# michaelfeil/skyjo_rl

Measured on AMD Instinct MI355X. Metric: env-steps/sec (whole node) at 65 536 parallel 3-player games, higher is better.
Workload: dtype int8

## Files before the change

skyjo_rl_amd/csrc/skyjo_step.h:

```cpp
#pragma once
#ifndef SKYJO_DEVICE_PARTS
#error "include skyjo_device.h"
#endif

__device__ __forceinline__ void sk_publish_deals(const SkParams &P, int g) {
  const size_t G = (size_t)P.tiles * SK_TILE;
  const int b = P.busy[g];
  if (b) {
    const uint32_t tag = P.plan_tag[g];
    const uint32_t f = __hip_atomic_load(&P.done_flag[g], __ATOMIC_RELAXED, __HIP_MEMORY_SCOPE_AGENT);
    if ((f & 0x7fffffffu) == tag) {
      SK_FENCE_ACQUIRE(P);
      if (!P.cancel[g] && f == tag) P.spare_ready[(size_t)(b - 1) * G + g] = 1;
      P.busy[g] = 0, P.cancel[g] = 0;
    }
  }
}
__device__ __forceinline__ void sk_plan_deals(const SkParams &P, int g, int lane) {
  const size_t G = (size_t)P.tiles * SK_TILE;
  bool need = false, empty = false;
  if (g < P.B) {
    const uint8_t busy = P.busy[g];
    const int head = P.bank_head[g] % SK_BANK;
    const uint32_t consumed = P.deals_consumed[g];
    uint8_t ready[SK_BANK];
#pragma unroll
    for (int k = 0; k < SK_BANK; k++) ready[k] = P.spare_ready[(size_t)k * G + g];
    bool open = true;
    int r = 0;
#pragma unroll
    for (int k = 0; k < SK_BANK; k++) {
      uint8_t f = 0;
#pragma unroll
      for (int j = 0; j < SK_BANK; j++) f = (head + k) % SK_BANK == j ? ready[j] : f;
      open = open && f != 0;
      r += open ? 1 : 0;
    }
    need = !busy && r < SK_BANK;
    empty = need && r == 0;
    if (need) {
      P.busy[g] = (uint8_t)(1 + (head + r) % SK_BANK);
      P.cancel[g] = 0;
      P.plan_ep[g] = consumed + (uint32_t)r;
      P.plan_tag[g] = P.plan_new_tag;
    }
  }
  const unsigned long long be = __ballot(empty);
  if (be && lane == 0) atomicAdd(P.bank_empty + (P.be_add & 1u), (uint32_t)__popcll(be));
}

__device__ __forceinline__ void sk_error_to_host(const SkParams &P, int lane) {
  if (lane == 0) {
    const uint32_t e = __hip_atomic_load(P.dev_error, __ATOMIC_RELAXED, __HIP_MEMORY_SCOPE_AGENT);
    if (e) P.health_host[2] = e;
  }
}
__device__ __forceinline__ void sk_export_raw(const SkParams &P, uint8_t *lp, int g, uint8_t *o) {
  for (int c = 0; c < P.L.chunks; c++) ((uint4 *)o)[c] = LQ(c);
  double *d = (double *)(o + P.L.state_bytes);
  for (int p = 0; p < P.L.N; p++) d[p] = P.rewards[(size_t)g * P.L.N + p], d[P.L.N + p] = P.scores[(size_t)g * P.L.N + p];
  uint32_t *m = (uint32_t *)(d + 2 * P.L.N);
  m[0] = P.rng_mode == SKYJO_RNG_MT19937 ? (uint32_t)P.mt_idx[g] : 0u;
  m[1] = P.done[g];
}

__device__ __forceinline__ uint32_t sk_next_tag(uint32_t t) {
  t = (t + 1u) & 0x7fffffffu;
  return t ? t : 1u;
}
template <bool INDIRECT, bool POLICY, int NP, bool PLANAR = false>
__device__ __forceinline__ void step_body(const SkParams &Pin, const int tile, const int lane, uint32_t *lds_raw, const int32_t *actions,
                                          uint8_t *rec_out, int32_t *act_out, int iters, uint64_t policy_seed, uint64_t iter0,
                                          double *end_rew_out, uint8_t *end_out, uint8_t *raw_out, int raw_stride, const int cycle_len = 0,
                                          const bool defer_ok = true) {
  SkParams P = Pin;
  TRACE_DECL;
  if (NP > 0) P.L = sk_make_layout(NP, INDIRECT ? 1 : 0);
  const int g = tile * SK_TILE + lane;
  const uint32_t lds_tile = (uint32_t)(uintptr_t)(__attribute__((address_space(3))) uint32_t *)lds_raw;
  uint8_t *lp = (uint8_t *)lds_raw + lane * 16;
  uint8_t *stg = (uint8_t *)lds_raw + P.L.chunks * 1024;
  uint8_t *fp = stg + lane * 4;
  const int stg_bytes = (INDIRECT || PLANAR) ? 4096 : SK_TILE * (P.L.rec_bytes + 16);
  uint8_t *ap = stg + stg_bytes + lane * 8;
  constexpr bool DEFER = POLICY && NP > 0 && NP < 8;
  constexpr bool REGACC = NP > 0 && NP < 8;
  constexpr int NACC = REGACC ? SK_ACC_KINDS * NP : 1;
  double racc_store[NACC];
#pragma unroll
  for (int k = 0; k < NACC; k++) racc_store[k] = 0.0;
  double *racc = REGACC ? racc_store : nullptr;
  uint8_t *pendp = DEFER && defer_ok ? stg + stg_bytes + (REGACC ? 0 : SK_ACC_KINDS * P.L.N * 512) + lane * 16 : nullptr;
  int pend_fin = -1;
  if (!REGACC)
    for (int k = 0; k < SK_ACC_KINDS * P.L.N; k++) ACC(k) = 0.0;
  STAMP_DECL;
  if (!POLICY) tile_load(P, P.state, tile, lane, lp);
  else dma_record<true>((const uint8_t *)P.state, (uint32_t)((((size_t)tile * P.L.chunks) * SK_TILE + lane) * 16), lds_tile, P.L.chunks);
  if (P.ov_flags & 1u) sk_publish_deals(P, g);
  sk_vm_drain();
  HdrRegs h;
  HDR_LOAD(h);
  STAMP(0);
  const bool valid = ((h.w0 >> 16) & F_VALID) != 0;
  LaneCounters cnt;
  uint32_t r0 = 0, r1 = 0, r2 = 0, r3 = 0;
  const uint64_t gid = P.game_id0 + (uint64_t)g;
  ObsRegs ob;
  if (valid) obs_load(P, lp, (h.w0 >> 8) & 0xff, ob);
  for (int it = 0; it < iters; it++) {
    const uint64_t iter = iter0 + (uint64_t)it;
    if (POLICY && (it == 0 || (iter & 3) == 0)) {
      philox4x32_10((uint32_t)(iter >> 2), (uint32_t)gid, (uint32_t)(gid >> 32), 0x504F4C00u, (uint32_t)policy_seed,
                    (uint32_t)(policy_seed >> 32), r0, r1, r2, r3);
      for (int k = (int)(iter & 3); k > 0; k--) {
        const uint32_t t = r0;
        r0 = r1, r1 = r2, r2 = r3, r3 = t;
      }
    }
    STAMP_T(3);
    const uint32_t word = r0;
    if (POLICY) {
      r0 = r1, r1 = r2, r2 = r3, r3 = word;
    }
    int a = -1;
    if (valid) {
      const bool over = ((h.w0 >> 16) & F_DONE) != 0;
      if (!POLICY) a = actions[g];
      const bool skip = !POLICY && a == SKYJO_ACTION_SKIP;
      const bool acted = !over && !skip;
      SpareRegs sp;
      const bool resetting = over && P.auto_reset && !skip;
      if (resetting) spare_issue(P, lp, lds_tile, tile, lane, g, sp);
      STAMP_T(4);
      if (!over && !skip) {
        const uint32_t v0 = ob.q0, v1 = ob.q1, v2 = ob.q2;
        STAMP_N(2);
        const uint4 row_pre = LQ(sk_pb(P.L, (h.w0 >> 8) & 0xff) >> 4);
        asm volatile("" ::: "memory");
        if (POLICY) a = policy_pick(h.w0 & 0xff, ob, word);
#ifndef SK_STAMPS_FINE
        STAMP_N(3);
#endif
        apply_action<INDIRECT, NP, POLICY>(P, lp, fp, ap, h, v0, v1, v2, a, g, cnt, st, pendp, pend_fin, row_pre, racc);
#ifdef SK_STAMPS_FINE
        STAMP(6);
#else
        STAMP(5);
#endif
      } else if (!skip) {
        a = -1;
        if (P.auto_reset) {
          bool dealt = true;
          if (!spare_commit(P, lp, g, sp)) {
            dealt = deal_inline(P, lp, fp, g, tile, lane, sp.head);
            cnt.waits++;
          }
          HDR_LOAD(h);
          if (SK_OFTEN(dealt)) {
            h.w0 = (h.w0 & 0x00ffffffu) | ((uint32_t)SKYJO_ST_RESET << 24);
            cnt.resets++;
          }
        } else {
          h.w0 = (h.w0 & 0x00ffffffu) | ((uint32_t)SKYJO_ST_NOOP_DONE << 24);
        }
        STAMP(1);
      } else {
        a = -1;
      }
      if (!POLICY && acted && (unsigned)a >= (unsigned)SKYJO_NUM_ACTIONS) a = -2;
      if (!POLICY && end_out) {
        const bool end = acted && ((h.w0 >> 16) & F_DONE) != 0;
        end_out[g] = end ? 1 : 0;
        for (int q = 0; q < P.L.N; q++) end_rew_out[(size_t)g * P.L.N + q] = end ? P.rewards[(size_t)g * P.L.N + q] : 0.0;
      }
      const uint4 rec_a = LQ(1);
      const uint32_t rec_b = LB(32);
      const uint4 rec_row = LQ((sk_pb(P.L, (h.w0 >> 8) & 0xff) + PB_VIS) >> 4);
      asm volatile("" ::: "memory");
      obs_from_row(rec_row, ob);
      if (rec_out) {
        if (INDIRECT) {
          uint4 rr[4];
          emit_record<INDIRECT>(P, lp, h, ob, a, nullptr, rr, &rec_a, rec_b);
          if (PLANAR) {
            typedef uint32_t u32x4_t __attribute__((ext_vector_type(4)));
            uint8_t *blk = rec_out + ((size_t)it * P.tiles + (size_t)tile) * (SK_TILE * 64) + lane * 16;
#pragma unroll
            for (int p = 0; p < 4; p++) __builtin_nontemporal_store((u32x4_t){rr[p].x, rr[p].y, rr[p].z, rr[p].w}, (u32x4_t *)(blk + p * 1024));
          } else {
#pragma unroll
            for (int p = 0; p < 4; p++) *(uint4 *)(stg + lane * 64 + ((p + (lane >> 1)) & 3) * 16) = rr[p];
          }
        } else if (PLANAR) {
          constexpr int PIECES = NP > 0 ? (((19 + 12 * NP + 3) & ~3) + 32 + 15) / 16 : 1;
          uint32_t wbuf[4 * PIECES];
#pragma unroll
          for (int k = 0; k < 4 * PIECES; k++) wbuf[k] = 0u;
          emit_record<INDIRECT>(P, lp, h, ob, a, (uint8_t *)wbuf, nullptr, &rec_a, rec_b);
          typedef uint32_t u32x4_t __attribute__((ext_vector_type(4)));
          uint8_t *blk = rec_out + ((size_t)it * P.tiles + (size_t)tile) * (SK_TILE * 16 * PIECES) + lane * 16;
#pragma unroll
          for (int p = 0; p < PIECES; p++)
            __builtin_nontemporal_store((u32x4_t){wbuf[4 * p], wbuf[4 * p + 1], wbuf[4 * p + 2], wbuf[4 * p + 3]}, (u32x4_t *)(blk + p * 1024));
        } else {
          emit_record<INDIRECT>(P, lp, h, ob, a, stg + lane * sk_stage_stride(P.L.rec_bytes), nullptr, &rec_a, rec_b);
        }
      }
      if (act_out) __builtin_nontemporal_store(a, &act_out[(size_t)it * P.B + g]);
#ifdef SK_STAMPS_FINE
      STAMP(7);
#else
      STAMP(6);
#endif
    }
    if (DEFER && ((it & (SK_SCORE_EVERY - 1)) == SK_SCORE_EVERY - 1 || it == iters - 1)) {
      if (SK_RARE(__any(pend_fin >= 0))) {
        if (pend_fin >= 0) {
          finish_game_fixed<(NP > 0 && NP < 8) ? NP : 1>(P, pendp, 1024, ap, g, pend_fin, racc);
          pend_fin = -1;
        }
      }
    }
    if (!INDIRECT && !PLANAR && rec_out) {
      typedef uint32_t u32x4_t __attribute__((ext_vector_type(4)));
      const int pieces = P.L.rec_bytes >> 4, stride = sk_stage_stride(P.L.rec_bytes);
      uint8_t *blk = rec_out + ((size_t)it * P.B + (size_t)tile * SK_TILE) * (size_t)P.L.rec_bytes;
      const int live = P.B - tile * SK_TILE;
      for (int q0 = lane; q0 < pieces * SK_TILE; q0 += 4 * SK_TILE) {
        uint4 v[4];
#pragma unroll
        for (int j = 0; j < 4; j++) {
          const int q = q0 + j * SK_TILE, r = q / pieces, p = q - r * pieces;
          if (q < pieces * SK_TILE) v[j] = *(const uint4 *)(stg + r * stride + p * 16);
        }
        if (SK_OFTEN(live >= SK_TILE)) {
#pragma unroll
          for (int j = 0; j < 4; j++) {
            const int q = q0 + j * SK_TILE;
            if (q0 - lane + j * SK_TILE < pieces * SK_TILE)
              __builtin_nontemporal_store((u32x4_t){v[j].x, v[j].y, v[j].z, v[j].w}, (u32x4_t *)(blk + (size_t)q * 16));
          }
        } else {
#pragma unroll
          for (int j = 0; j < 4; j++) {
            const int q = q0 + j * SK_TILE, r = q / pieces;
            if (q < pieces * SK_TILE && r < live)
              __builtin_nontemporal_store((u32x4_t){v[j].x, v[j].y, v[j].z, v[j].w}, (u32x4_t *)(blk + (size_t)q * 16));
          }
        }
      }
    }
    if (INDIRECT && !PLANAR && rec_out) {
      typedef uint32_t u32x4_t __attribute__((ext_vector_type(4)));
      uint8_t *blk = rec_out + ((size_t)it * P.B + (size_t)tile * SK_TILE) * 64;
      const int live = P.B - tile * SK_TILE;
      uint4 v[4];
#pragma unroll
      for (int j = 0; j < 4; j++) {
        const int r = 16 * j + (lane >> 2), p = lane & 3;
        v[j] = *(const uint4 *)(stg + r * 64 + ((p + (r >> 1)) & 3) * 16);
      }
      if (SK_OFTEN(live >= SK_TILE)) {
#pragma unroll
        for (int j = 0; j < 4; j++)
          __builtin_nontemporal_store((u32x4_t){v[j].x, v[j].y, v[j].z, v[j].w}, (u32x4_t *)(blk + j * 1024 + lane * 16));
      } else {
#pragma unroll
        for (int j = 0; j < 4; j++)
          if (16 * j + (lane >> 2) < live)
            __builtin_nontemporal_store((u32x4_t){v[j].x, v[j].y, v[j].z, v[j].w}, (u32x4_t *)(blk + j * 1024 + lane * 16));
      }
    }
    STAMP_T(2);
    if (POLICY && cycle_len && it + 1 < iters && (it + 1) % cycle_len == 0) {
      if (P.busy[g]) (void)wait_deal_done(P, g);
      sk_publish_deals(P, g);
      sk_plan_deals(P, g, lane);
      P.plan_new_tag = sk_next_tag(P.plan_new_tag);
      TRACE_WAIT_BEGIN;
      __syncthreads();
      TRACE_WAIT_END;
    }
  }
  HDR_FLUSH(h);
  tile_store_nt(P, P.state, tile, lane, lp);
  if (!POLICY && raw_out && valid) sk_export_raw(P, lp, g, raw_out + (size_t)g * raw_stride);
  if (P.ov_flags & 2u) {
    if (P.ov_flags & 1u) {
      if (P.busy[g]) (void)wait_deal_done(P, g);
      sk_publish_deals(P, g);
    }
    sk_plan_deals(P, g, lane);
  }
  if (!POLICY) {
    sk_error_to_host(P, lane);
    if (P.host_seq) {
      __threadfence_system();
      if (lane == 0) __hip_atomic_store(&P.health_host[3], P.host_seq, __ATOMIC_RELEASE, __HIP_MEMORY_SCOPE_SYSTEM);
    }
  }
  uint32_t v[7] = {cnt.steps, cnt.episodes, cnt.illegal, cnt.resets, cnt.sum_len, cnt.reshuffles, cnt.waits};
#pragma unroll
  for (int k = 0; k < 7; k++)
    for (int off = 32; off > 0; off >>= 1) v[k] += __shfl_down(v[k], off, 64);
  if (lane == 0) {
    unsigned long long *c = P.tile_counters + (size_t)tile * 8;
#pragma unroll
    for (int k = 0; k < 7; k++) c[k] += v[k];
  }
  if (__any(cnt.episodes | cnt.illegal)) {
    double mine = 0.0;
    if (REGACC) {
#pragma unroll
      for (int k = 0; k < NACC; k++) {
        double x = racc_store[k];
        for (int off = 32; off > 0; off >>= 1) x += __shfl_down(x, off, 64);
        x = __shfl(x, 0, 64);
        mine = lane == k ? x : mine;
      }
    } else {
      for (int k = 0; k < SK_ACC_KINDS * P.L.N; k++) {
        double x = ACC(k);
        for (int off = 32; off > 0; off >>= 1) x += __shfl_down(x, off, 64);
        x = __shfl(x, 0, 64);
        mine = lane == k ? x : mine;
      }
    }
    if (lane < SK_ACC_KINDS * P.L.N)
      P.acc_tile[(size_t)tile * SK_ACC_KINDS * SKYJO_MAX_PLAYERS + (lane / P.L.N) * SKYJO_MAX_PLAYERS + lane % P.L.N] += mine;
  }
  STAMP(7);
  STAMP_STORE;
  TRACE_STORE(0, (uint32_t)(iter0 / (uint64_t)(iters > 0 ? iters : 1)), lane, tile);
}

template <bool INDIRECT, bool POLICY, int NP, bool PLANAR = false>
__global__ __launch_bounds__(SK_TILE) void k_step(SkParams Pin, const int32_t *actions, uint8_t *rec_out,
                                                  int32_t *act_out, int iters, uint64_t policy_seed, uint64_t iter0,
                                                  double *end_rew_out, uint8_t *end_out, uint8_t *raw_out, int raw_stride) {
  extern __shared__ uint32_t lds_raw[];
  step_body<INDIRECT, POLICY, NP, PLANAR>(Pin, (int)blockIdx.x, (int)threadIdx.x, lds_raw, actions, rec_out, act_out, iters, policy_seed, iter0,
                                          end_rew_out, end_out, raw_out, raw_stride);
}

template <bool INDIRECT>
__device__ __forceinline__ void sk_emit_to(const SkParams &P, uint8_t *lp, const HdrRegs &h, const ObsRegs &ob, uint8_t *rec_out, int tile, int lane,
                                           int planar) {
  const int g = tile * SK_TILE + lane;
  if (INDIRECT && planar) {
    uint4 rr[4];
    emit_record<INDIRECT>(P, lp, h, ob, -1, nullptr, rr);
    uint4 *o = (uint4 *)(rec_out + (size_t)tile * SK_TILE * P.L.rec_bytes) + lane;
#pragma unroll
    for (int k = 0; k < 4; k++) o[k * SK_TILE] = rr[k];
  } else {
    emit_record<INDIRECT>(P, lp, h, ob, -1, rec_out + (size_t)g * P.L.rec_bytes);
  }
}

template <bool INDIRECT>
__global__ __launch_bounds__(SK_TILE) void k_observe(SkParams P, const int32_t *players, uint8_t *rec_out, int planar) {
  extern __shared__ uint32_t lds_raw[];
  const int tile = blockIdx.x, lane = threadIdx.x, g = tile * SK_TILE + lane;
  uint8_t *lp = (uint8_t *)lds_raw + lane * 16;
  sk_error_to_host(P, lane);
  tile_load(P, P.state, tile, lane, lp);
  if (!(LB(H_FLAGS) & F_VALID)) return;
  HdrRegs h;
  HDR_LOAD(h);
  int q = players ? players[g] : LB(H_PLAYER);
  q = q < 0 ? 0 : (q >= P.L.N ? P.L.N - 1 : q);
  ObsRegs ob;
  obs_load(P, lp, q, ob);
  sk_emit_to<INDIRECT>(P, lp, h, ob, rec_out, tile, lane, planar);
}

template <bool INDIRECT>
__global__ __launch_bounds__(SK_TILE) void k_reset(SkParams P, const uint8_t *mask, uint8_t *rec_out, uint8_t *raw_out, int raw_stride, int planar) {
  extern __shared__ uint32_t lds_raw[];
  const int tile = blockIdx.x, lane = threadIdx.x, g = tile * SK_TILE + lane;
  uint8_t *lp = (uint8_t *)lds_raw + lane * 16;
  uint8_t *fp = (uint8_t *)lds_raw + P.L.chunks * 1024 + lane * 4;
  if (g >= P.B) return;
  const bool want = !mask || mask[g];
  bool want_counted = false;
  tile_load(P, P.state, tile, lane, lp);
  if (want) {
    const int head = P.bank_head[g] % SK_BANK;
    bool dealt = true;
    if (!consume_spare(P, lp, tile, lane, g, head)) dealt = deal_inline(P, lp, fp, g, tile, lane, head);
    if (dealt) LB(H_STATUS) = SKYJO_ST_RESET;
    want_counted = dealt;
  }
  HdrRegs h;
  HDR_LOAD(h);
  if (rec_out) {
    ObsRegs ob;
    obs_load(P, lp, LB(H_PLAYER), ob);
    sk_emit_to<INDIRECT>(P, lp, h, ob, rec_out, tile, lane, planar);
  }
  if (want) tile_store(P, P.state, tile, lane, lp);
  if (raw_out && (LB(H_FLAGS) & F_VALID)) sk_export_raw(P, lp, g, raw_out + (size_t)g * raw_stride);
  sk_error_to_host(P, lane);
  const unsigned long long wb = __ballot(want_counted);
  if (want_counted && lane == __ffsll((long long)wb) - 1) P.tile_counters[(size_t)tile * 8 + 3] += __popcll(wb);
}
```

skyjo_rl_amd/csrc/skyjo_transition.h:

```cpp
#pragma once
#ifndef SKYJO_DEVICE_PARTS
#error "include skyjo_device.h"
#endif

__device__ __forceinline__ void refresh_minima(const SkParams &P, uint8_t *lp) {
  int ms = LSH(sk_pb(P.L, 0) + PB_SUM), mh = LB(sk_pb(P.L, 0) + PB_HIDDEN);
  for (int q = 1; q < P.L.N; q++) {
    int s = LSH(sk_pb(P.L, q) + PB_SUM), h = LB(sk_pb(P.L, q) + PB_HIDDEN);
    ms = s < ms ? s : ms, mh = h < mh ? h : mh;
  }
  LB(H_MINSUM) = (uint8_t)(int8_t)(ms < 127 ? ms : 127);
  LB(H_MINHID) = (uint8_t)mh;
}

template <class Rng>
__device__ __forceinline__ void reshuffle_discard(const SkParams &P, uint8_t *lp, Rng &r) {
  const int n = LB(H_NDISC), role = LB(H_ROLE), pb = P.L.off_pile;
  const int reg = role ? 0 : 1;
  for (int i = n - 1; i >= 1; i--) {
    int j = (int)rng_interval(r, (uint32_t)i);
    int ai = pb + pile_addr(reg, i), aj = pb + pile_addr(reg, j);
    uint8_t t = LB(ai);
    LB(ai) = LB(aj), LB(aj) = t;
  }
  for (int k = 0; k < n - 1; k++) LB(H_HIST + 2 + LI(pb + pile_addr(reg, k)))--;
  int last = LI(pb + pile_addr(reg, n - 1));
  LB(pb + pile_addr(reg ^ 1, 0)) = (uint8_t)last;
  LB(H_NDRAW) = (uint8_t)(n - 1), LB(H_NDISC) = 1, LB(H_ROLE) = (uint8_t)(role ^ 1);
  LB(H_TOP) = (uint8_t)last;
  int rs = LB(H_RESH);
  LB(H_RESH) = (uint8_t)(rs < 255 ? rs + 1 : 255);
}

#define SK_WAIT_OK 0
#define SK_WAIT_GAVE_UP 1
#define SK_WAIT_TIMEOUT 2
__device__ __forceinline__ int wait_deal_done(const SkParams &P, int g) {
  uint32_t f = 0;
  const uint32_t tag = P.plan_tag[g];
  for (int spin = 0; spin < (1 << P.spin_log2); spin++) {
    f = __hip_atomic_load(&P.done_flag[g], __ATOMIC_RELAXED, __HIP_MEMORY_SCOPE_AGENT);
    if ((f & 0x7fffffffu) == tag) break;
    __builtin_amdgcn_s_sleep(32);
  }
  if ((f & 0x7fffffffu) != tag) {
    atomicOr(P.dev_error, SK_ERR_DEAL_TIMEOUT);
    return SK_WAIT_TIMEOUT;
  }
  SK_FENCE_ACQUIRE(P);
  return (f >> 31) != 0 ? SK_WAIT_GAVE_UP : SK_WAIT_OK;
}

__device__ __forceinline__ uint32_t mt_untwist_y(const uint32_t *mt, int i) {
  uint32_t t = mt[i] ^ mt[i + 397 >= 624 ? i + 397 - 624 : i + 397];
  const uint32_t odd = t >> 31;
  t ^= odd ? 0x9908b0dfu : 0u;
  return (t << 1) | odd;
}
__device__ __forceinline__ void mt_untwist(uint32_t *mt, int from, int to) {
  for (int i = to; i != from;) {
    const int nx = i == 624 ? 0 : i;
    i = nx == 0 ? 623 : nx - 1;
    const uint32_t y = mt_untwist_y(mt, i);
    const int ip1 = i == 623 ? 0 : i + 1;
    mt[ip1] = (mt[ip1] & 0x80000000u) | (y & 0x7fffffffu);
    mt[i] = y & 0x80000000u;
  }
}

__device__ __forceinline__ int mt_rollback(const SkParams &P, uint32_t *mt, int g, int slot, int packed) {
  const size_t G = (size_t)P.tiles * SK_TILE;
  const int snap = P.mt_idx[(size_t)(1 + slot) * G + g];
  int from = (snap & 0xffff) + (snap >> 16), to = (packed & 0xffff) + (packed >> 16);
  from = from >= 624 ? from - 624 : from, to = to >= 624 ? to - 624 : to;
  mt_untwist(mt, from, to);
  return snap;
}

__device__ __forceinline__ void reshuffle_dispatch(const SkParams &P, uint8_t *lp, uint8_t *fp, int g) {
  if (P.rng_mode == SKYJO_RNG_MT19937) {
    const size_t G = (size_t)P.tiles * SK_TILE;
    uint32_t *mt = P.mt + (size_t)g * 624;
    const int head = LB(H_BANK) % SK_BANK;
    const int busy = P.busy[g];
    const bool inflight = busy && !P.cancel[g];
    bool undo_inflight = false;
    if (inflight) {
      const int w = wait_deal_done(P, g);
      if (w == SK_WAIT_TIMEOUT) {
        LB(H_FLAGS) |= F_DONE, LB(H_STATUS) = SKYJO_ST_ERROR, LB(H_NDRAW) = 1;
        P.done[g] = 1;
        for (int q = 0; q < P.L.N; q++) P.rewards[(size_t)g * P.L.N + q] = 0.0;
        return;
      }
      undo_inflight = w == SK_WAIT_OK;
      P.cancel[g] = 1;
    }
    int packed = P.mt_idx[g];
    if (undo_inflight) packed = mt_rollback(P, mt, g, busy - 1, packed);
    for (int k = SK_BANK - 1; k >= 0; k--) {
      const int slot = (head + k) % SK_BANK;
      if (P.spare_ready[(size_t)slot * G + g]) {
        packed = mt_rollback(P, mt, g, slot, packed);
        P.spare_ready[(size_t)slot * G + g] = 0;
      }
    }
    MtStream<16> r;
    r.open(mt, packed, fp);
    reshuffle_discard(P, lp, r);
    P.mt_idx[g] = r.close();
  } else {
    PhiloxStream r;
    r.open(P.seeds[g] + 1, *(uint32_t *)(lp + LIDX(H_EPISODE)), LB(H_RESH), 1u);
    reshuffle_discard(P, lp, r);
  }
}

#define ACC(k) (*(double *)(ap + ((k) << 9)))
__device__ __forceinline__ void acc_add(uint8_t *ap, int k, double v) {
  __hip_atomic_fetch_add(&ACC(k), v, __ATOMIC_RELAXED, __HIP_MEMORY_SCOPE_WAVEFRONT);
}
__device__ __forceinline__ void acc_episode(uint8_t *ap, int N, int p, double score, double reward, int refunded) {
  acc_add(ap, p, score), acc_add(ap, N + p, reward), acc_add(ap, 2 * N + p, reward * reward);
  if (refunded) acc_add(ap, 3 * N + p, (double)refunded);
}

__device__ __forceinline__ void finish_game(const SkParams &P, uint8_t *lp, uint8_t *fp, uint8_t *ap, int g,
                                            int finisher) {
  const int N = P.L.N;
  double *sc = P.scores + (size_t)g * N, *rw = P.rewards + (size_t)g * N;
  int mn = 0, fs = 0;
  for (int p = 0; p < N; p++) {
    int s = 0;
    for (int c = 0; c < 4; c++) {
      int b = sk_pb(P.L, p) + PB_CARDS + 3 * c;
      int t0 = LI(b), t1 = LI(b + 1), t2 = LI(b + 2);
      if (!(t0 == t1 && t1 == t2)) s += t0 + t1 + t2;
    }
    MT_FIFO(p) = (uint32_t)s;
    mn = (p == 0 || s < mn) ? s : mn;
    fs = p == finisher ? s : fs;
  }
  const bool penal = mn != fs;
#define SCORE(p) ((penal && (p) == finisher) ? (double)(int)MT_FIFO(p) * P.score_penalty : (double)(int)MT_FIFO(p))
  double sum;
  if (N < 8) {
    sum = 0.0;
    for (int p = 0; p < N; p++) sum += SCORE(p);
  } else {
    sum = ((SCORE(0) + SCORE(1)) + (SCORE(2) + SCORE(3))) + ((SCORE(4) + SCORE(5)) + (SCORE(6) + SCORE(7)));
    for (int p = 8; p < N; p++) sum += SCORE(p);
  }
  const double mean = sum / (double)N;
  for (int p = 0; p < N; p++) {
    const double d = SCORE(p);
    double r = (-d + mean) + P.mean_reward;
    const int rf = LB(sk_pb(P.L, p) + PB_REFUNDED);
    if (P.reward_refunded != 0.0) r += (double)rf * P.reward_refunded;
    sc[p] = d, rw[p] = r;
    acc_episode(ap, N, p, d, r, rf);
  }
#undef SCORE
  P.done[g] = 1;
}

template <int NP>
__device__ __forceinline__ void finish_game_fixed(const SkParams &P, const uint8_t *rows, int stride, uint8_t *ap, int g, int finisher,
                                                  double *racc = nullptr) {
  double *sc = P.scores + (size_t)g * NP, *rw = P.rewards + (size_t)g * NP;
  int s[NP], refunded[NP];
  int mn = 0, fs = 0;
#pragma unroll
  for (int p = 0; p < NP; p++) {
    const uint4 row = *(const uint4 *)(rows + p * stride);
    const uint32_t c0 = row.x, c1 = row.y, c2 = row.z;
    refunded[p] = (int)(row.w >> 24);
    const uint32_t tri[4] = {c0 & 0xffffffu, (c0 >> 24) | ((c1 & 0xffffu) << 8), (c1 >> 16) | ((c2 & 0xffu) << 16), c2 >> 8};
    int t = 0;
#pragma unroll
    for (int c = 0; c < 4; c++) {
      const int t0 = (int)(int8_t)tri[c], t1 = (int)(int8_t)(tri[c] >> 8), t2 = (int)(int8_t)(tri[c] >> 16);
      t += (t0 == t1 && t1 == t2) ? 0 : t0 + t1 + t2;
    }
    s[p] = t;
    mn = (p == 0 || t < mn) ? t : mn;
    fs = p == finisher ? t : fs;
  }
  const bool penal = mn != fs;
  double d[NP], sum = 0.0;
#pragma unroll
  for (int p = 0; p < NP; p++) {
    d[p] = (penal && p == finisher) ? (double)s[p] * P.score_penalty : (double)s[p];
    sum += d[p];
  }
  const double mean = sum / (double)NP;
#pragma unroll
  for (int p = 0; p < NP; p++) {
    double r = (-d[p] + mean) + P.mean_reward;
    if (P.reward_refunded != 0.0) r += (double)refunded[p] * P.reward_refunded;
    sc[p] = d[p], rw[p] = r;
    if (racc) {
      racc[p] += d[p], racc[NP + p] += r, racc[2 * NP + p] += r * r, racc[3 * NP + p] += (double)refunded[p];
    } else {
      acc_episode(ap, NP, p, d[p], r, refunded[p]);
    }
  }
}

struct HdrRegs {
  uint32_t w0, w1, w2;
};
#define HDR_LOAD(h) ((h).w0 = LW(0), (h).w1 = LW(1), (h).w2 = LW(2))
#define HDR_FLUSH(h) (LW(0) = (h).w0, LW(1) = (h).w1, LW(2) = (h).w2)

__device__ __forceinline__ int byte3(uint32_t a, uint32_t b, uint32_t c, int k) {
  const uint32_t w = k < 4 ? a : (k < 8 ? b : c);
  return (int)(int8_t)(w >> ((k & 3) * 8));
}
__device__ __forceinline__ void put3(uint32_t &a, uint32_t &b, uint32_t &c, int k, int val) {
  const uint32_t sh = (uint32_t)(k & 3) * 8u, m = ~(0xffu << sh), v = ((uint32_t)val & 0xffu) << sh;
  if (k < 4) a = (a & m) | v;
  else if (k < 8) b = (b & m) | v;
  else c = (c & m) | v;
}
__device__ __forceinline__ void hist_add(uint8_t *lp, int value, int delta) {
  const int b = H_HIST + 2 + value;
  uint32_t *w = (uint32_t *)(lp + LIDX(b & ~3));
  const uint32_t d = (uint32_t)delta << ((b & 3) * 8);
  __hip_atomic_fetch_add(w, d, __ATOMIC_RELAXED, __HIP_MEMORY_SCOPE_WAVEFRONT);
}
__device__ __forceinline__ uint32_t swar_nonzero01(uint32_t x) {
  return ((((x & 0x7f7f7f7fu) + 0x7f7f7f7fu) | x) & 0x80808080u) >> 7;
}
__device__ __forceinline__ uint32_t pack12(uint32_t a, uint32_t b, uint32_t c) {
  return ((a * 0x00204081u >> 21) & 0xfu) | (((b * 0x00204081u >> 21) & 0xfu) << 4) |
         (((c * 0x00204081u >> 21) & 0xfu) << 8);
}

struct ObsRegs {
  uint32_t q0, q1, q2, nz0, nz1, nz2, hd0, hd1, hd2;
};
__device__ __forceinline__ void obs_from_row(const uint4 &row, ObsRegs &o) {
  o.q0 = row.x, o.q1 = row.y, o.q2 = row.z;
  o.nz0 = swar_nonzero01(o.q0 ^ 0xf2f2f2f2u);
  o.nz1 = swar_nonzero01(o.q1 ^ 0xf2f2f2f2u);
  o.nz2 = swar_nonzero01(o.q2 ^ 0xf2f2f2f2u);
  o.hd0 = swar_nonzero01(o.q0 ^ 0x0f0f0f0fu) ^ 0x01010101u;
  o.hd1 = swar_nonzero01(o.q1 ^ 0x0f0f0f0fu) ^ 0x01010101u;
  o.hd2 = swar_nonzero01(o.q2 ^ 0x0f0f0f0fu) ^ 0x01010101u;
}
__device__ __forceinline__ void obs_load(const SkParams &P, uint8_t *lp, int q, ObsRegs &o) {
  const uint4 row = LQ((sk_pb(P.L, q) + PB_VIS) >> 4);
  obs_from_row(row, o);
}

__device__ __forceinline__ int policy_pick(int phase, const ObsRegs &o, uint32_t word) {
  if (phase == 0) return 24 + (int)__umulhi(word, 2u);
  uint32_t legal = pack12(o.nz0, o.nz1, o.nz2) | (pack12(o.hd0, o.hd1, o.hd2) << 12);
  const int n = __popc(legal);
  if (n == 0) return 24;
  int k = (int)__umulhi(word, (uint32_t)n), pos = 0;
  int c = __popc(legal & 0xfffu);
  if (k >= c) k -= c, pos = 12, legal >>= 12;
  c = __popc(legal & 0x3fu);
  if (k >= c) k -= c, pos += 6, legal >>= 6;
  c = __popc(legal & 0x7u);
  if (k >= c) k -= c, pos += 3, legal >>= 3;
  c = (int)(legal & 1u);
  if (k >= c) {
    k -= c, pos += 1;
    c = (int)((legal >> 1) & 1u);
    if (k >= c) pos += 1;
  }
  return pos;
}

template <bool INDIRECT, int NP, bool TRUSTED>
__device__ __forceinline__ void apply_action(const SkParams &P, uint8_t *lp, uint8_t *fp, uint8_t *ap, HdrRegs &h, uint32_t v0,
                                             uint32_t v1, uint32_t v2, int a, int g, LaneCounters &cnt, Stamps &st,
                                             uint8_t *pendp, int &pend_fin, const uint4 &row_pre, double *racc = nullptr) {
  const int N = P.L.N;
  const int phase = h.w0 & 0xff, p = (h.w0 >> 8) & 0xff;
  const int blk = sk_pb(P.L, p), cardb = blk + PB_CARDS, visb = blk + PB_VIS, pb = P.L.off_pile;
  const unsigned ua = (unsigned)a;
  int slot = 0, sv = 0;
  bool legal;
  if (ua < 24u) {
    slot = a < 12 ? a : a - 12;
    sv = byte3(v0, v1, v2, slot);
    legal = phase == 1 && (TRUSTED || (a < 12 ? sv != SKYJO_REFUNDED : sv == SKYJO_HAND_NONE));
  } else {
    legal = (TRUSTED || ua <= 25u) && phase == 0;
  }
  if (!legal) {
    double *rw = P.rewards + (size_t)g * N;
    for (int q = 0; q < N; q++) rw[q] = q == p ? P.illegal_reward : 0.0;
    if (NP > 0 && racc) {
#pragma unroll
      for (int q = 0; q < (NP > 0 ? NP : 1); q++)
        racc[NP + q] += q == p ? P.illegal_reward : 0.0, racc[2 * NP + q] += q == p ? P.illegal_reward * P.illegal_reward : 0.0;
    } else {
      acc_add(ap, N + p, P.illegal_reward), acc_add(ap, 2 * N + p, P.illegal_reward * P.illegal_reward);
    }
    h.w0 = (h.w0 & 0x0000ffffu) | ((((h.w0 >> 16) & 0xffu) | F_DONE) << 16) | ((uint32_t)SKYJO_ST_ILLEGAL << 24);
    P.done[g] = 1;
    cnt.illegal++;
    return;
  }
  const int eplen = (int)(h.w2 & 0xffffu) + 1;
  h.w2 = (h.w2 & 0xffff0000u) | (uint32_t)eplen;
  h.w0 &= 0x00ffffffu;
  cnt.steps++;
  if (phase == 0) {
    const int role = (h.w1 >> 16) & 1;
    int nd = h.w1 & 0xff;
    const int ns = (h.w1 >> 8) & 0xff;
    const int hidden_p = (int)((row_pre.w >> 16) & 0xffu);
    int pile_top = LI(pb + pile_addr(role, nd > 0 ? nd - 1 : 0));
    const int disc_top = LI(pb + pile_addr(role ^ 1, ns > 0 ? ns - 1 : 0));
    const int disc_below = LI(pb + pile_addr(role ^ 1, ns > 1 ? ns - 2 : 0));

    if (hidden_p == 0) {
      h.w0 |= (uint32_t)(F_TERMINATED | F_DONE) << 16;
      LB(H_FINISHER) = (uint8_t)p;
      if (NP > 0 && NP < 8) {
        constexpr int NQ = (NP > 0 && NP < 8) ? NP : 1;
        P.done[g] = 1;
        if (pendp) {
#pragma unroll
          for (int q = 0; q < NQ; q++) *(uint4 *)(pendp + q * 1024) = LQ(sk_pb(P.L, q) >> 4);
          pend_fin = p;
        } else {
          finish_game_fixed<NQ>(P, lp + (P.L.off_players >> 4) * 1024, 2048, ap, g, p, racc);
        }
      } else {
        finish_game(P, lp, fp, ap, g, p);
      }
      cnt.episodes++;
      cnt.sum_len += eplen;
#ifdef SK_STAMPS_FINE
      STAMP(3);
#endif
      return;
    }
    const bool from_pile = a == 24;
    if (from_pile && nd == 0) {
      HDR_FLUSH(h);
      reshuffle_dispatch(P, lp, fp, g);
      HDR_LOAD(h);
      cnt.reshuffles++;
      nd = h.w1 & 0xff;
      pile_top = LI(pb + pile_addr((h.w1 >> 16) & 1, nd - 1));
    }
    int hand;
    if (from_pile) {
      hand = pile_top;
      h.w1 = (h.w1 & 0xffffff00u) | (uint32_t)(nd - 1);
    } else {
      hand = disc_top;
      hist_add(lp, hand, -1);
      const int top = ns > 1 ? disc_below : -3;
      h.w1 = (h.w1 & 0x00ff00ffu) | ((uint32_t)(ns - 1) << 8) | (((uint32_t)top & 0xffu) << 24);
    }
    h.w2 = (h.w2 & 0x00ffffffu) | (((uint32_t)hand & 0xffu) << 24);
    h.w0 = (h.w0 & 0xffffff00u) | 1u;
#ifdef SK_STAMPS_FINE
    STAMP(3);
#endif
    return;
  }
  STAMP_N(4);
  const int hand = (int)(int8_t)(h.w2 >> 24);
  const int reg = ((h.w1 >> 16) & 1) ^ 1;
  int ns = (h.w1 >> 8) & 0xff;
  const uint4 row = row_pre;
  const uint32_t c0 = row.x, c1 = row.y, c2 = row.z;
  int sum = (int)(int16_t)(row.w & 0xffffu), hid = (int)((row.w >> 16) & 0xffu), refunded = (int)(row.w >> 24);
  int oms = 1 << 20, omh = 1 << 20;
  for (int q = 0; q < N; q++) {
    const uint32_t cq = LW((sk_pb(P.L, q) + PB_SUM) >> 2);
    const int s = (int)(int16_t)(cq & 0xffffu), hq = (int)((cq >> 16) & 0xffu);
    oms = (q != p && s < oms) ? s : oms, omh = (q != p && hq < omh) ? hq : omh;
  }
#ifdef SK_STAMPS_FINE
  STAMP(5);
#endif
  const bool swap = a < 12, was_hidden = sv == SKYJO_HAND_NONE;
  const int under = byte3(c0, c1, c2, slot);
  const int shown = swap ? hand : under, gone = swap ? under : hand;
  LB(pb + pile_addr(reg, ns)) = (uint8_t)gone;
  ns++;
  hist_add(lp, gone, 1);
  LB(cardb + slot) = (uint8_t)shown;
  LB(visb + slot) = (uint8_t)shown;
  put3(v0, v1, v2, slot, shown);
  sum += shown - (was_hidden ? 0 : under);
  hid -= was_hidden ? 1 : 0;
  if (!INDIRECT) {
    if (!was_hidden) hist_add(lp, under, -1);
    hist_add(lp, shown, 1);
  }
  int top = gone;
  {
    const uint32_t tri[4] = {v0 & 0xffffffu, (v0 >> 24) | ((v1 & 0xffffu) << 8), (v1 >> 16) | ((v2 & 0xffu) << 16), v2 >> 8};
    bool full[4];
#pragma unroll
    for (int c = 0; c < 4; c++) {
      const uint32_t b0 = tri[c] & 0xffu;
      full[c] = ((tri[c] ^ (tri[c] >> 8)) & 0xffffu) == 0 && b0 != (uint32_t)SKYJO_HAND_NONE && b0 != ((uint32_t)SKYJO_REFUNDED & 0xffu);
    }
    if (full[0] | full[1] | full[2] | full[3]) {
#pragma unroll
      for (int c = 0; c < 4; c++)
        if (full[c]) {
          const int t0 = (int)(int8_t)(tri[c] & 0xff);
          for (int k = 0; k < 3; k++) {
            LB(cardb + 3 * c + k) = (uint8_t)(int8_t)SKYJO_REFUNDED;
            LB(visb + 3 * c + k) = (uint8_t)(int8_t)SKYJO_REFUNDED;
            LB(pb + pile_addr(reg, ns)) = 0;
            ns++;
          }
          hist_add(lp, 0, 3);
          if (!INDIRECT) hist_add(lp, t0, -3);
          sum -= 3 * t0;
          top = 0;
        }
      refunded++;
    }
  }
  LW((blk + PB_SUM) >> 2) = ((uint32_t)sum & 0xffffu) | ((uint32_t)hid << 16) | ((uint32_t)refunded << 24);
  __hip_atomic_fetch_add((uint32_t *)(lp + LIDX(blk + PB_PLACED)), 1u, __ATOMIC_RELAXED, __HIP_MEMORY_SCOPE_WAVEFRONT);
  const int ms = sum < oms ? sum : oms, mh = hid < omh ? hid : omh;
  LB(H_MINSUM) = (uint8_t)(int8_t)(ms < 127 ? ms : 127);
  LB(H_MINHID) = (uint8_t)mh;
  h.w1 = (h.w1 & 0x00ff00ffu) | ((uint32_t)ns << 8) | (((uint32_t)top & 0xffu) << 24);
  h.w2 = (h.w2 & 0x00ffffffu) | ((uint32_t)SKYJO_HAND_NONE << 24);
  const int np = p + 1 == N ? 0 : p + 1;
  h.w0 = (h.w0 & 0xffff0000u) | ((uint32_t)np << 8);
}
```

Measured before the change: 47.91 billion.

## Specialize step loop per wavefront phase via ballot for uniform-phase waves

```diff
diff --git a/skyjo_rl_amd/csrc/skyjo_step.h b/skyjo_rl_amd/csrc/skyjo_step.h
--- a/skyjo_rl_amd/csrc/skyjo_step.h
+++ b/skyjo_rl_amd/csrc/skyjo_step.h
@@ -125,99 +125,42 @@
     }
     int a = -1;
     if (valid) {
-      const bool over = ((h.w0 >> 16) & F_DONE) != 0;
-      if (!POLICY) a = actions[g];
-      const bool skip = !POLICY && a == SKYJO_ACTION_SKIP;
-      const bool acted = !over && !skip;
-      SpareRegs sp;
-      const bool resetting = over && P.auto_reset && !skip;
-      if (resetting) spare_issue(P, lp, lds_tile, tile, lane, g, sp);
-      STAMP_T(4);
-      if (!over && !skip) {
-        const uint32_t v0 = ob.q0, v1 = ob.q1, v2 = ob.q2;
-        STAMP_N(2);
-        const uint4 row_pre = LQ(sk_pb(P.L, (h.w0 >> 8) & 0xff) >> 4);
-        asm volatile("" ::: "memory");
-        if (POLICY) a = policy_pick(h.w0 & 0xff, ob, word);
-#ifndef SK_STAMPS_FINE
-        STAMP_N(3);
+#ifdef SK_NO_PAIR
+      if (false) {
+#else
+      if (POLICY && NP > 0) {
 #endif
-        apply_action<INDIRECT, NP, POLICY>(P, lp, fp, ap, h, v0, v1, v2, a, g, cnt, st, pendp, pend_fin, row_pre, racc);
-#ifdef SK_STAMPS_FINE
-        STAMP(6);
-#else
-        STAMP(5);
+        const bool draws = (h.w0 & (0xffu | ((uint32_t)F_DONE << 16))) == 0;
+        const unsigned long long b_draw = __ballot(draws), b_other = __ballot(!draws);
+#ifndef SK_B0
+#define SK_B0 1
 #endif
-      } else if (!skip) {
-        a = -1;
-        if (P.auto_reset) {
-          bool dealt = true;
-          if (!spare_commit(P, lp, g, sp)) {
-            dealt = deal_inline(P, lp, fp, g, tile, lane, sp.head);
-            cnt.waits++;
-          }
-          HDR_LOAD(h);
-          if (SK_OFTEN(dealt)) {
-            h.w0 = (h.w0 & 0x00ffffffu) | ((uint32_t)SKYJO_ST_RESET << 24);
-            cnt.resets++;
-          }
+#ifndef SK_B1
+#define SK_B1 1
+#endif
+        if (SK_B0 && b_other == 0) {
+#define SK_PH 0
+#include "skyjo_step_iter.h"
+#undef SK_PH
+        } else if (SK_B1 && SK_OFTEN(b_draw == 0)) {
+#define SK_PH 1
+#include "skyjo_step_iter.h"
+#undef SK_PH
         } else {
-          h.w0 = (h.w0 & 0x00ffffffu) | ((uint32_t)SKYJO_ST_NOOP_DONE << 24);
+#define SK_PH -1
+#include "skyjo_step_iter.h"
+#undef SK_PH
         }
-        STAMP(1);
       } else {
-        a = -1;
-      }
-      if (!POLICY && acted && (unsigned)a >= (unsigned)SKYJO_NUM_ACTIONS) a = -2;
-      if (!POLICY && end_out) {
-        const bool end = acted && ((h.w0 >> 16) & F_DONE) != 0;
-        end_out[g] = end ? 1 : 0;
-        for (int q = 0; q < P.L.N; q++) end_rew_out[(size_t)g * P.L.N + q] = end ? P.rewards[(size_t)g * P.L.N + q] : 0.0;
-      }
-      const uint4 rec_a = LQ(1);
-      const uint32_t rec_b = LB(32);
-      const uint4 rec_row = LQ((sk_pb(P.L, (h.w0 >> 8) & 0xff) + PB_VIS) >> 4);
-      asm volatile("" ::: "memory");
-      obs_from_row(rec_row, ob);
-      if (rec_out) {
-        if (INDIRECT) {
-          uint4 rr[4];
-          emit_record<INDIRECT>(P, lp, h, ob, a, nullptr, rr, &rec_a, rec_b);
-          if (PLANAR) {
-            typedef uint32_t u32x4_t __attribute__((ext_vector_type(4)));
-            uint8_t *blk = rec_out + ((size_t)it * P.tiles + (size_t)tile) * (SK_TILE * 64) + lane * 16;
-#pragma unroll
-            for (int p = 0; p < 4; p++) __builtin_nontemporal_store((u32x4_t){rr[p].x, rr[p].y, rr[p].z, rr[p].w}, (u32x4_t *)(blk + p * 1024));
-          } else {
-#pragma unroll
-            for (int p = 0; p < 4; p++) *(uint4 *)(stg + lane * 64 + ((p + (lane >> 1)) & 3) * 16) = rr[p];
-          }
-        } else if (PLANAR) {
-          constexpr int PIECES = NP > 0 ? (((19 + 12 * NP + 3) & ~3) + 32 + 15) / 16 : 1;
-          uint32_t wbuf[4 * PIECES];
-#pragma unroll
-          for (int k = 0; k < 4 * PIECES; k++) wbuf[k] = 0u;
-          emit_record<INDIRECT>(P, lp, h, ob, a, (uint8_t *)wbuf, nullptr, &rec_a, rec_b);
-          typedef uint32_t u32x4_t __attribute__((ext_vector_type(4)));
-          uint8_t *blk = rec_out + ((size_t)it * P.tiles + (size_t)tile) * (SK_TILE * 16 * PIECES) + lane * 16;
-#pragma unroll
-          for (int p = 0; p < PIECES; p++)
-            __builtin_nontemporal_store((u32x4_t){wbuf[4 * p], wbuf[4 * p + 1], wbuf[4 * p + 2], wbuf[4 * p + 3]}, (u32x4_t *)(blk + p * 1024));
-        } else {
-          emit_record<INDIRECT>(P, lp, h, ob, a, stg + lane * sk_stage_stride(P.L.rec_bytes), nullptr, &rec_a, rec_b);
-        }
-      }
-      if (act_out) __builtin_nontemporal_store(a, &act_out[(size_t)it * P.B + g]);
-#ifdef SK_STAMPS_FINE
-      STAMP(7);
-#else
-      STAMP(6);
-#endif
+#define SK_PH -1
+#include "skyjo_step_iter.h"
+#undef SK_PH
+      }
     }
     if (DEFER && ((it & (SK_SCORE_EVERY - 1)) == SK_SCORE_EVERY - 1 || it == iters - 1)) {
       if (SK_RARE(__any(pend_fin >= 0))) {
         if (pend_fin >= 0) {
-          finish_game_fixed<(NP > 0 && NP < 8) ? NP : 1>(P, pendp, 1024, ap, g, pend_fin, racc);
+          finish_game_fixed<(NP > 0 && NP < 8) ? NP : 1, true>(P, pendp, 1024, ap, g, pend_fin, racc);
           pend_fin = -1;
         }
       }
diff --git a/skyjo_rl_amd/csrc/skyjo_step_iter.h b/skyjo_rl_amd/csrc/skyjo_step_iter.h
--- /dev/null
+++ b/skyjo_rl_amd/csrc/skyjo_step_iter.h
@@ -0,0 +1,99 @@
+#ifndef SK_PH
+#error "skyjo_step_iter.h is included by skyjo_step.h with SK_PH defined"
+#endif
+#if SK_PH == 0
+      const bool over = false;
+#else
+      const bool over = ((h.w0 >> 16) & F_DONE) != 0;
+#endif
+      if (!POLICY) a = actions[g];
+      const bool skip = !POLICY && a == SKYJO_ACTION_SKIP;
+      const bool acted = !over && !skip;
+      SpareRegs sp;
+      const bool resetting = over && P.auto_reset && !skip;
+      if (resetting) spare_issue(P, lp, lds_tile, tile, lane, g, sp);
+      STAMP_T(4);
+      if (!over && !skip) {
+        const uint32_t v0 = ob.q0, v1 = ob.q1, v2 = ob.q2;
+        STAMP_N(2);
+        const uint4 row_pre = LQ(sk_pb(P.L, (h.w0 >> 8) & 0xff) >> 4);
+        asm volatile("" ::: "memory");
+        if (POLICY) a = policy_pick<SK_PH>(h.w0 & 0xff, ob, word);
+#ifndef SK_STAMPS_FINE
+        STAMP_N(3);
+#endif
+        apply_action<INDIRECT, NP, POLICY, SK_PH>(P, lp, fp, ap, h, v0, v1, v2, a, g, cnt, st, pendp, pend_fin, row_pre, racc);
+#ifdef SK_STAMPS_FINE
+        STAMP(6);
+#else
+        STAMP(5);
+#endif
+      } else if (!skip) {
+        a = -1;
+        if (P.auto_reset) {
+          bool dealt = true;
+          if (!spare_commit(P, lp, g, sp)) {
+            dealt = deal_inline(P, lp, fp, g, tile, lane, sp.head);
+            cnt.waits++;
+          }
+          HDR_LOAD(h);
+          if (SK_OFTEN(dealt)) {
+            h.w0 = (h.w0 & 0x00ffffffu) | ((uint32_t)SKYJO_ST_RESET << 24);
+            cnt.resets++;
+          }
+        } else {
+          h.w0 = (h.w0 & 0x00ffffffu) | ((uint32_t)SKYJO_ST_NOOP_DONE << 24);
+        }
+        STAMP(1);
+      } else {
+        a = -1;
+      }
+      if (!POLICY && acted && (unsigned)a >= (unsigned)SKYJO_NUM_ACTIONS) a = -2;
+      if (!POLICY && end_out) {
+        const bool end = acted && ((h.w0 >> 16) & F_DONE) != 0;
+        end_out[g] = end ? 1 : 0;
+        for (int q = 0; q < P.L.N; q++) end_rew_out[(size_t)g * P.L.N + q] = end ? P.rewards[(size_t)g * P.L.N + q] : 0.0;
+      }
+      const uint4 rec_a = LQ(1);
+      const uint32_t rec_b = LB(32);
+#if SK_PH == 0
+      asm volatile("" ::: "memory");
+#else
+      const uint4 rec_row = LQ((sk_pb(P.L, (h.w0 >> 8) & 0xff) + PB_VIS) >> 4);
+      asm volatile("" ::: "memory");
+      obs_from_row(rec_row, ob);
+#endif
+      if (rec_out) {
+        if (INDIRECT) {
+          uint4 rr[4];
+          emit_record<INDIRECT>(P, lp, h, ob, a, nullptr, rr, &rec_a, rec_b);
+          if (PLANAR) {
+            typedef uint32_t u32x4_t __attribute__((ext_vector_type(4)));
+            uint8_t *blk = rec_out + ((size_t)it * P.tiles + (size_t)tile) * (SK_TILE * 64) + lane * 16;
+#pragma unroll
+            for (int p = 0; p < 4; p++) __builtin_nontemporal_store((u32x4_t){rr[p].x, rr[p].y, rr[p].z, rr[p].w}, (u32x4_t *)(blk + p * 1024));
+          } else {
+#pragma unroll
+            for (int p = 0; p < 4; p++) *(uint4 *)(stg + lane * 64 + ((p + (lane >> 1)) & 3) * 16) = rr[p];
+          }
+        } else if (PLANAR) {
+          constexpr int PIECES = NP > 0 ? (((19 + 12 * NP + 3) & ~3) + 32 + 15) / 16 : 1;
+          uint32_t wbuf[4 * PIECES];
+#pragma unroll
+          for (int k = 0; k < 4 * PIECES; k++) wbuf[k] = 0u;
+          emit_record<INDIRECT>(P, lp, h, ob, a, (uint8_t *)wbuf, nullptr, &rec_a, rec_b);
+          typedef uint32_t u32x4_t __attribute__((ext_vector_type(4)));
+          uint8_t *blk = rec_out + ((size_t)it * P.tiles + (size_t)tile) * (SK_TILE * 16 * PIECES) + lane * 16;
+#pragma unroll
+          for (int p = 0; p < PIECES; p++)
+            __builtin_nontemporal_store((u32x4_t){wbuf[4 * p], wbuf[4 * p + 1], wbuf[4 * p + 2], wbuf[4 * p + 3]}, (u32x4_t *)(blk + p * 1024));
+        } else {
+          emit_record<INDIRECT>(P, lp, h, ob, a, stg + lane * sk_stage_stride(P.L.rec_bytes), nullptr, &rec_a, rec_b);
+        }
+      }
+      if (act_out) __builtin_nontemporal_store(a, &act_out[(size_t)it * P.B + g]);
+#ifdef SK_STAMPS_FINE
+      STAMP(7);
+#else
+      STAMP(6);
+#endif
diff --git a/skyjo_rl_amd/csrc/skyjo_transition.h b/skyjo_rl_amd/csrc/skyjo_transition.h
--- a/skyjo_rl_amd/csrc/skyjo_transition.h
+++ b/skyjo_rl_amd/csrc/skyjo_transition.h
@@ -164,7 +164,7 @@
   P.done[g] = 1;
 }
 
-template <int NP>
+template <int NP, bool REGS = false>
 __device__ __forceinline__ void finish_game_fixed(const SkParams &P, const uint8_t *rows, int stride, uint8_t *ap, int g, int finisher,
                                                   double *racc = nullptr) {
   double *sc = P.scores + (size_t)g * NP, *rw = P.rewards + (size_t)g * NP;
@@ -199,7 +199,7 @@
     double r = (-d[p] + mean) + P.mean_reward;
     if (P.reward_refunded != 0.0) r += (double)refunded[p] * P.reward_refunded;
     sc[p] = d[p], rw[p] = r;
-    if (racc) {
+    if (REGS) {
       racc[p] += d[p], racc[NP + p] += r, racc[2 * NP + p] += r * r, racc[3 * NP + p] += (double)refunded[p];
     } else {
       acc_episode(ap, NP, p, d[p], r, refunded[p]);
@@ -254,8 +254,9 @@
   obs_from_row(row, o);
 }
 
+template <int PH = -1>
 __device__ __forceinline__ int policy_pick(int phase, const ObsRegs &o, uint32_t word) {
-  if (phase == 0) return 24 + (int)__umulhi(word, 2u);
+  if (PH == 0 || (PH < 0 && phase == 0)) return 24 + (int)__umulhi(word, 2u);
   uint32_t legal = pack12(o.nz0, o.nz1, o.nz2) | (pack12(o.hd0, o.hd1, o.hd2) << 12);
   const int n = __popc(legal);
   if (n == 0) return 24;
@@ -275,17 +276,19 @@
   return pos;
 }
 
-template <bool INDIRECT, int NP, bool TRUSTED>
+template <bool INDIRECT, int NP, bool TRUSTED, int PH = -1>
 __device__ __forceinline__ void apply_action(const SkParams &P, uint8_t *lp, uint8_t *fp, uint8_t *ap, HdrRegs &h, uint32_t v0,
                                              uint32_t v1, uint32_t v2, int a, int g, LaneCounters &cnt, Stamps &st,
                                              uint8_t *pendp, int &pend_fin, const uint4 &row_pre, double *racc = nullptr) {
   const int N = P.L.N;
-  const int phase = h.w0 & 0xff, p = (h.w0 >> 8) & 0xff;
+  const int phase = PH >= 0 ? PH : (int)(h.w0 & 0xff), p = (h.w0 >> 8) & 0xff;
   const int blk = sk_pb(P.L, p), cardb = blk + PB_CARDS, visb = blk + PB_VIS, pb = P.L.off_pile;
   const unsigned ua = (unsigned)a;
   int slot = 0, sv = 0;
   bool legal;
-  if (ua < 24u) {
+  if (TRUSTED && PH == 0) {
+    legal = true;
+  } else if (ua < 24u) {
     slot = a < 12 ? a : a - 12;
     sv = byte3(v0, v1, v2, slot);
     legal = phase == 1 && (TRUSTED || (a < 12 ? sv != SKYJO_REFUNDED : sv == SKYJO_HAND_NONE));
@@ -295,7 +298,7 @@
   if (!legal) {
     double *rw = P.rewards + (size_t)g * N;
     for (int q = 0; q < N; q++) rw[q] = q == p ? P.illegal_reward : 0.0;
-    if (NP > 0 && racc) {
+    if (NP > 0 && NP < 8) {
 #pragma unroll
       for (int q = 0; q < (NP > 0 ? NP : 1); q++)
         racc[NP + q] += q == p ? P.illegal_reward : 0.0, racc[2 * NP + q] += q == p ? P.illegal_reward * P.illegal_reward : 0.0;
@@ -331,7 +334,7 @@
           for (int q = 0; q < NQ; q++) *(uint4 *)(pendp + q * 1024) = LQ(sk_pb(P.L, q) >> 4);
           pend_fin = p;
         } else {
-          finish_game_fixed<NQ>(P, lp + (P.L.off_players >> 4) * 1024, 2048, ap, g, p, racc);
+          finish_game_fixed<NQ, true>(P, lp + (P.L.off_players >> 4) * 1024, 2048, ap, g, p, racc);
         }
       } else {
         finish_game(P, lp, fp, ap, g, p);
```

Result: slower. 42.06 billion (-12.2%).
